# Bricktricker/gpu-solve

Measured on AMD Instinct MI355X. Metric: MLUPS (Jacobi smoother) + V-cycle wall-time, 512³ fp64; achieved HBM GB/s %peak, higher is better.
Workload: dtype f64

## Files before the change

gpu-solve_amd/csrc/gs_device.hpp:

```cpp
#pragma once
#include <hip/hip_runtime.h>
#include <math.h>

#include <cmath>
#include <stdint.h>
#include <stdlib.h>

#include <map>
#include <mutex>
#include <utility>

#include "gpusolve_hip.h"

#ifdef GS_EXP_NOEXP
#define exp(x) ((x) * 1.0000001)
#endif
#ifdef GS_EXP_NOBAR
#define GS_LDS_BARRIER() __builtin_amdgcn_s_waitcnt(0xc07f)
#else
#define GS_LDS_BARRIER()                                                                                               \
    do {                                                                                                               \
        __builtin_amdgcn_s_waitcnt(0xc07f);                                                                            \
        __builtin_amdgcn_s_barrier();                                                                                  \
    } while (0)
#endif

namespace {

constexpr int WAVE = 64;

constexpr bool newtonish(int m) { return m == GS_NEWTON || m == GS_NEWTON_B; }
constexpr int base_mode(int m) { return m == GS_NEWTON_G ? GS_NEWTON_B : m; }

template <bool B>
struct BoolC {
    __device__ static constexpr bool get() { return B; }
};
struct RtBool {
    bool b;
    __device__ bool get() const { return b; }
};

struct Coef {
    double s[7];
    double hh;
    double omega[3];
    double gamma;
    double alpha;
    double preFac;
    int fastdiv;
    int unit;
    int swz;
    int zq;
    int bconst;
    int64_t off[7];
#ifdef GS_EXP_EFIELD
    int64_t efoff;
#endif
};

bool canonical_order(const gs_stencil* S)
{
    static const int cx[7] = {0, 1, -1, 0, 0, 0, 0};
    static const int cy[7] = {0, 0, 0, 1, -1, 0, 0};
    static const int cz[7] = {0, 0, 0, 0, 0, 1, -1};
    for (int i = 0; i < 7; i++)
        if (S->ox[i] != cx[i] || S->oy[i] != cy[i] || S->oz[i] != cz[i]) return false;
    return true;
}

bool valid_stencil(const gs_stencil* S)
{
    for (int i = 0; i < 7; i++)
        if (S->ox[i] < -1 || S->ox[i] > 1 || S->oy[i] < -1 || S->oy[i] > 1 || S->oz[i] < -1 || S->oz[i] > 1)
            return false;
    return true;
}

struct Knobs {
    bool unitStencil, tbxPfd2, pairXh, fitRounds, bigChunks, oneRound, rrLds, zeroQ, newtonXh, specCached;
    int xhSwizzle, midZc, rrZc, rrZcBig, oneRoundMid, rbZc;
    int slabZc, pairZc, rrNr, rrNtu, rrReverse, rrNg, rrDma;
    bool pairFx;
    int fmgNt;
    int64_t pairMinBlocks;
    static int num(const char* name, int dflt)
    {
        const char* e = getenv(name);
        return e && *e ? atoi(e) : dflt;
    }
    Knobs()
        : unitStencil(getenv("GS_NO_UNIT_STENCIL") == nullptr), tbxPfd2(num("GS_TBX_PFD", 2) != 1),
          pairXh(num("GS_PAIR_XH", 1) != 0), fitRounds(num("GS_FIT_ROUNDS", 1) != 0),
          bigChunks(num("GS_PAIR_BIG_CHUNKS", 1) != 0), oneRound(num("GS_PAIR_ONE_ROUND", 1) != 0),
          rrLds(getenv("GS_RR_LDS") != nullptr), zeroQ(getenv("GS_NO_ZERO_Q") == nullptr),
          newtonXh(num("GS_NEWTON_XH", 1) != 0), specCached(num("GS_SPEC_CACHED", 0) != 0),
          xhSwizzle(num("GS_XH_SWIZZLE", 1)), midZc(num("GS_MID_ZC", 0)), rrZc(num("GS_RR_ZC", 0)), rrZcBig(num("GS_RR_ZC_BIG", 0)), oneRoundMid(num("GS_PAIR_ONE_ROUND_MID", 0)), rbZc(num("GS_RB_ZC", 0)), slabZc(num("GS_SLAB_ZC", 0)), pairZc(num("GS_PAIR_ZC", 0)),
          rrNr(num("GS_RR_NR", 0)), rrNtu(num("GS_RR_NTU", 2)), rrReverse(num("GS_RR_REVERSE", 1)), rrNg(num("GS_RR_NG", 0)), rrDma(num("GS_RR_DMA", 0)),
          pairFx(num("GS_PAIR_FX", 1) != 0), fmgNt(num("GS_FMG_NT", -1)),
          pairMinBlocks(num("GS_PAIR_MIN_BLOCKS", 128))
    {
    }
};
const Knobs kKnobs;

#ifdef GS_EXP_EFIELD
int64_t gs_exp_efoff = 0;
#endif

Coef make_coef(const gs_stencil* S, const gs_level* L, double omega, double gamma, int bconst = 0)
{
    Coef k;
    for (int i = 0; i < 7; i++) {
        k.s[i] = S->s[i];
        k.off[i] = S->ox[i] + S->oy[i] * L->ldy + S->oz[i] * L->ldz;
    }
    k.hh = L->h * L->h;
    for (int i = 0; i < 3; i++) k.omega[i] = omega;
    k.gamma = gamma;
    k.alpha = k.hh / S->s[0];
    k.preFac = S->s[0] / k.hh;
    k.fastdiv = k.hh >= 0x1p-120 && k.hh <= 1.0;
    k.unit = kKnobs.unitStencil && (S->s[0] >= 1.0 || S->s[0] <= -1.0);
    for (int i = 1; i < 7; i++) k.unit = k.unit && S->s[i] == -1.0;
    k.swz = kKnobs.xhSwizzle;
    k.zq = kKnobs.zeroQ && std::isnormal(k.hh) && k.hh > 0.0;
    for (int i = 0; i < 7; i++) k.zq = k.zq && std::isfinite(S->s[i]);
    k.bconst = bconst;
#ifdef GS_EXP_EFIELD
    k.efoff = gs_exp_efoff;
#endif
    return k;
}

Coef make_coef_w(const gs_stencil* S, const gs_level* L, const double* omegas, int n, double gamma, int bconst = 0)
{
    Coef k = make_coef(S, L, omegas[0], gamma, bconst);
    for (int i = 1; i < 3; i++) k.omega[i] = omegas[i < n ? i : n - 1];
    return k;
}


__device__ __forceinline__ double hh_recip(double hh)
{
    const double y0 = __builtin_amdgcn_rcp(hh);
    const double y1 = __builtin_fma(y0, __builtin_fma(-hh, y0, 1.0), y0);
    return __builtin_fma(y1, __builtin_fma(-hh, y1, 1.0), y1);
}

__device__ __forceinline__ double div_hh(const Coef& k, double s)
{
    const unsigned e = ((unsigned)__double2hiint(s) >> 20) & 0x7ffu;
    if (k.fastdiv && e - 124u < 1500u) {
        const double y = hh_recip(k.hh);
        const double q = s * y;
        const double r = __builtin_fma(-k.hh, q, s);
        return __builtin_fma(r, y, q);
    }
    return s / k.hh;
}

__device__ __forceinline__ bool div_hh_fast_ok(double s)
{
    const unsigned e = ((unsigned)__double2hiint(s) >> 20) & 0x7ffu;
    return e - 124u < 1500u;
}
template <int N>
__device__ __forceinline__ void div_hh_n(const Coef& k, double (&s)[N])
{
    bool ok = k.fastdiv;
#pragma unroll
    for (int i = 0; i < N; i++) ok &= div_hh_fast_ok(s[i]);
    if (ok) {
        const double y = hh_recip(k.hh);
#pragma unroll
        for (int i = 0; i < N; i++) {
            const double q = s[i] * y;
            const double r = __builtin_fma(-k.hh, q, s[i]);
            s[i] = __builtin_fma(r, y, q);
        }
    } else {
#pragma unroll
// ... 166 lines not shown
    return MODE == GS_NEWTON_B ? 1.0 : exp(w);
}

__device__ __forceinline__ double wave_sum(double x)
{
#pragma unroll
    for (int o = WAVE / 2; o > 0; o >>= 1) x += __shfl_down(x, o, WAVE);
    return x;
}

template <int NWAVES>
__device__ __forceinline__ double block_sum(double x, double* lds, int nw = NWAVES)
{
    const int tid = threadIdx.x + threadIdx.y * blockDim.x;
    x = wave_sum(x);
    if ((tid & (WAVE - 1)) == 0) lds[tid / WAVE] = x;
    __syncthreads();
    double t = 0.0;
    if (tid == 0) {
#pragma unroll
        for (int i = 0; i < NWAVES; i++)
            if (i < nw) t += lds[i];
    }
    return t;
}

template <bool DPP>
__device__ __forceinline__ double lane_from_left(double src, double edge)
{
    if (DPP) {
        const long long s = __double_as_longlong(src), e = __double_as_longlong(edge);
        const int lo = __builtin_amdgcn_update_dpp((int)e, (int)s, 0x138, 0xf, 0xf, false);
        const int hi = __builtin_amdgcn_update_dpp((int)(e >> 32), (int)(s >> 32), 0x138, 0xf, 0xf, false);
        return __longlong_as_double(((long long)hi << 32) | (unsigned)lo);
    } else {
        const double t = __shfl_up(src, 1, WAVE);
        return (threadIdx.x & (WAVE - 1)) == 0 ? edge : t;
    }
}

template <bool DPP>
__device__ __forceinline__ double lane_from_right(double src, double edge)
{
    if (DPP) {
        const long long s = __double_as_longlong(src), e = __double_as_longlong(edge);
        const int lo = __builtin_amdgcn_update_dpp((int)e, (int)s, 0x130, 0xf, 0xf, false);
        const int hi = __builtin_amdgcn_update_dpp((int)(e >> 32), (int)(s >> 32), 0x130, 0xf, 0xf, false);
        return __longlong_as_double(((long long)hi << 32) | (unsigned)lo);
    } else {
        const double t = __shfl_down(src, 1, WAVE);
        return (threadIdx.x & (WAVE - 1)) == WAVE - 1 ? edge : t;
    }
}

__device__ __forceinline__ double uniform_d(double x)
{
    const long long b = __double_as_longlong(x);
    const int lo = __builtin_amdgcn_readfirstlane((int)b), hi = __builtin_amdgcn_readfirstlane((int)(b >> 32));
    return __longlong_as_double(((long long)(unsigned)hi << 32) | (unsigned)lo);
}

__device__ __forceinline__ double2 ld2(const double* __restrict__ p) { return *reinterpret_cast<const double2*>(p); }

typedef double dv2 __attribute__((ext_vector_type(2)));
template <bool NT>
__device__ __forceinline__ double2 ld2s(const double* __restrict__ p)
{
    if (NT) {
        const dv2 t = __builtin_nontemporal_load(reinterpret_cast<const dv2*>(p));
        return make_double2(t.x, t.y);
    }
    return ld2(p);
}
template <bool NT>
__device__ __forceinline__ void st2s(double* __restrict__ p, double a, double b)
{
    if (NT) {
        const dv2 t = {a, b};
        __builtin_nontemporal_store(t, reinterpret_cast<dv2*>(p));
    } else {
        *reinterpret_cast<double2*>(p) = make_double2(a, b);
    }
}

template <bool ZV, bool NT = false>
__device__ __forceinline__ double2 ldv2(const double* __restrict__ p)
{
    if (ZV) return make_double2(0.0, 0.0);
    return ld2s<NT>(p);
}
template <bool ZV>
__device__ __forceinline__ double ldv1(const double* __restrict__ p)
{
    return ZV ? 0.0 : *p;
}

__device__ __forceinline__ int64_t xcd_tile(int64_t b, int64_t nb)
{
    const int64_t q = nb / 8, r = nb % 8, x = b % 8, k = b / 8;
    return (x < r ? x * (q + 1) : r * (q + 1) + (x - r) * q) + k;
}

template <int MODE, int KIND, bool ADD, int RY, int W, bool DPP, bool NT = false, bool XCD = false, bool NTV = false,
          bool ZV = false, bool UN = false>
__global__ __launch_bounds__(WAVE* W) void k_rb(Coef k, const double* __restrict__ v, const double* __restrict__ f,
                                                 const double* __restrict__ w, double* __restrict__ out,
                                                 double* __restrict__ partials, int nx, int ny, int nz, int64_t ldy,
                                                 int64_t ldz, int ZC)
{
    __shared__ double red[W];
    const int lane = threadIdx.x;
    const int wv = __builtin_amdgcn_readfirstlane(threadIdx.y);
    int bx = blockIdx.x, by = blockIdx.y, bz = blockIdx.z;
    int64_t tile = blockIdx.x + gridDim.x * ((int64_t)blockIdx.y + gridDim.y * (int64_t)blockIdx.z);
    if (XCD) {
        const int nbx = (nx + 2 * WAVE - 1) / (2 * WAVE), nby = (ny + RY * W - 1) / (RY * W);
        tile = xcd_tile(blockIdx.x, gridDim.x);
        bx = (int)(tile % nbx);
        by = (int)((tile / nbx) % nby);
        bz = (int)(tile / ((int64_t)nbx * nby));
    }
    const int x0 = 1 + bx * (2 * WAVE);
    const int x = x0 + 2 * lane;
    const int xl = min(x, nx + 1);
    const int y0 = 1 + (by * W + wv) * RY;
    const int zb = 1 + bz * ZC;
    const int ze = min(zb + ZC - 1, nz);
    const int xle = x0 - 1;
    const int xre = min(x0 + 2 * WAVE, nx + 1);
    const bool okx0 = x <= nx, okx1 = x + 1 <= nx;
    const double* fin = (KIND == 2) ? out : f;

    int64_t roff[RY + 2];
#pragma unroll
    for (int r = 0; r < RY + 2; r++) roff[r] = (int64_t)min(y0 - 1 + r, ny + 1) * ldy;

    double2 P[RY], C[RY], NL[2][RY], FL[2][RY], WL[2][RY], HL[2][2];
    double EL[2][RY], ER[2][RY];
    double sumsq = 0.0;
    auto load_slot = [&](const int s, const int64_t z1, const int64_t z2) {
#pragma unroll
        for (int r = 0; r < RY; r++) {
            NL[s][r] = ldv2<ZV, NTV>(v + xl + roff[r + 1] + z2);
            if (KIND != 2 || ADD) FL[s][r] = ld2s<NT>(fin + xl + roff[r + 1] + z1);
            if (newtonish(MODE)) WL[s][r] = ld2(w + xl + roff[r + 1] + z1);
            EL[s][r] = ldv1<ZV>(v + xle + roff[r + 1] + z1);
            ER[s][r] = ldv1<ZV>(v + xre + roff[r + 1] + z1);
        }
        HL[s][0] = ldv2<ZV>(v + xl + roff[0] + z1);
        HL[s][1] = ldv2<ZV>(v + xl + roff[RY + 1] + z1);
    };
    if (zb <= ze) {
        const int64_t zo = (int64_t)zb * ldz;
#pragma unroll
        for (int r = 0; r < RY; r++) {
            P[r] = ldv2<ZV>(v + xl + roff[r + 1] + zo - ldz);
            C[r] = ldv2<ZV>(v + xl + roff[r + 1] + zo);
        }
        load_slot(1, zo, zo + ldz);
    }
    for (int z0 = zb; z0 <= ze; z0 += 2) {
#pragma unroll
        for (int ph = 0; ph < 2; ph++) {
            const int z = z0 + ph;
            const bool real = z <= ze;
            const int cs = ph ^ 1;
// ... 2180 lines not shown
                        }
                    }
                }
            };
            if constexpr (!SPEC) {
                sweeps(RtBool{mir});
            } else {
                if (mir) sweeps(BoolC<true>{});
                else sweeps(BoolC<false>{});
            }
#pragma unroll
            for (int j = 1; j <= RY; j++) {
                V1p[j - 1] = V1c[j];
                if (!RECOMP) Fprev[j - 1] = FL[cs][j];
                if constexpr (RECOMP) {
                    wprev_l[j - 1][wx + WX * wy][lane] = WL[cs][j];
                    fprev_l[j - 1][wx + WX * wy][lane] = FL[cs][j];
                } else if (newtonish(MODE)) {
                    Aprev[j - 1] = Acur[j - 1];
                    Eprev[j - 1] = Ecur[j - 1];
                }
            }
#pragma unroll
            for (int j = 0; j < NV; j++) {
                V1c[j] = V1n[j];
                Vp[j] = Vc[j];
                Vc[j] = VL[cs][j];
            }
            if constexpr (XH) {
                EP = EC;
                if constexpr (EPK) {
                    if (edg) EC = efld(cs, 0);
                } else {
                    EC = EA[cs];
                }
                ES1c = ES1n;
            }
            if (PRO && ph == 1) {
                if constexpr (WLDS) {
                    wsl ^= 1;
                } else {
#pragma unroll
                    for (int r = 0; r < NCR; r++) W0[r] = W1[r];
                    if constexpr (HALF) {
#pragma unroll
                        for (int r = 0; r < NCR; r++) H0[r] = H1[r];
                    }
                }
                xpass(1);
            }
        }
    }
    if (partials) {
        sumsq = wave_sum(sumsq);
        const int wid = wx + WX * wy;
        if (lane == 0) red[wid] = sumsq;
        __syncthreads();
        if (tid == 0) {
            double t = 0.0;
            for (int i = 0; i < 2 * WX; i++) t += red[i];
            partials[tile] = t;
        }
    }
    if constexpr (TS) {
        if (tid == 0) {
            double* t = const_cast<double*>(es) + 4 * tile;
            t[0] = (double)tstart;
            t[1] = (double)wall_clock64();
            t[2] = (double)(blockIdx.x + (int64_t)gridDim.x * blockIdx.y);
            t[3] = (double)(unsigned)__builtin_amdgcn_s_getreg((31 << 11) | 4);
        }
    }
}

constexpr int TBY_RY = 2, TBY_RY_NEWTON = 2, TBY_WX = 4, TB_RY_B = 2, TB_WX_B = 8;
constexpr int tby_pfd(int mode) { return mode == GS_LINEAR ? 2 : 1; }
bool tbx_pfd2() { return kKnobs.tbxPfd2; }

#ifdef GS_EXP_T3_CHAIN
#define GS_T3_ZP(n, c) c
#else
#define GS_T3_ZP(n, c) n
#endif
template <bool UN, bool FX, bool DB>
__global__ __launch_bounds__(WAVE* TBY_WX * 2) void k_tb3y(Coef k, const double* __restrict__ v,
                                                           const double* __restrict__ f, double* __restrict__ out,
                                                           int nx, int ny, int nz, int64_t ldy, int64_t ldz, int ZC)
{
    constexpr int MODE = GS_LINEAR, RY = TBY_RY, WXMAX = TBY_WX;
    static_assert(RY == 2, "k_tb3y: two rows per y-wave (the boundary tests below name the rows)");
    constexpr int N0 = RY + 2;
    constexpr int N1 = RY + 1;
    constexpr int NE = N0 + N1 + RY;
    constexpr int B1 = DB ? 2 : 1, B2 = DB ? N1 : 1, B3 = 1;
    __shared__ double edge[2][2][WXMAX + 2][2][NE];
    __shared__ double2 yrow[2][2][WXMAX][3][WAVE];
    __shared__ double2 f1_l[2][N1][2 * WXMAX][WAVE];
    __shared__ double2 f2_l[RY][2 * WXMAX][WAVE];
    __shared__ double2 s1p_l[N1][2 * WXMAX][WAVE];
    __shared__ double2 s2p_l[RY][2 * WXMAX][WAVE];
    const int lane = threadIdx.x;
    const int wy = __builtin_amdgcn_readfirstlane(threadIdx.z);
    const int WX = blockDim.y;
    const int wx = __builtin_amdgcn_readfirstlane(threadIdx.y);
    const int wid = wx + WXMAX * wy;
    const int tid = threadIdx.x + WAVE * (threadIdx.y + WX * threadIdx.z);
    for (int i = tid; i < 2 * 2 * (WXMAX + 2) * 2 * NE; i += WAVE * WX * 2) (&edge[0][0][0][0][0])[i] = 0.0;
    __syncthreads();
    const int64_t tile = xcd_tile(blockIdx.x + (int64_t)gridDim.x * blockIdx.y, (int64_t)gridDim.x * gridDim.y);
    const int x = 1 + wx * (2 * WAVE) + 2 * lane;
    const int xl = min(x, nx + 1);
    const bool bx0 = !FX && x > nx, bx1 = !FX && x + 1 > nx;
    const bool okx0 = FX || x <= nx, okx1 = FX || x + 1 <= nx;
    const int y0 = 1 + (int)(tile % gridDim.x) * (2 * RY);
    const int zb = 1 + (int)(tile / gridDim.x) * ZC;
    const int ze = min(zb + ZC - 1, nz);
    const bool mir = wy != 0;
    auto yof = [&](int j) { return mir ? y0 + 2 * RY - j : y0 - 1 + j; };

    int64_t roff[RY + 3];
    bool rowc[RY + 3];
#pragma unroll
    for (int j = -2; j <= RY; j++) {
        const int y = yof(j);
        roff[j + 2] = (int64_t)min(max(y, 0), ny + 1) * ldy;
        rowc[j + 2] = y >= 1 && y <= ny;
    }
    const bool in1 = rowc[1] && rowc[2] && rowc[3] && rowc[4];
    const bool in2 = rowc[2] && rowc[3] && rowc[4];
    auto planeok = [&](int z) { return z >= 1 && z <= nz; };
    auto cz = [&](int z) { return min(max(z, 0), nz + 1); };
    auto at = [&](const double* base, int j, int z) { return base + xl + roff[j + 2] + (int64_t)z * ldz; };

    double2 Vp[N0], Vc[N0], VL[2][N0], FL[2][N0], HL[2];
    double2 S1a[N0], S1c[N0], S2c[N1];
#pragma unroll
    for (int i = 0; i < N0; i++) S1a[i] = S1c[i] = make_double2(0.0, 0.0);
#pragma unroll
    for (int i = 0; i < N1; i++) {
        S2c[i] = make_double2(0.0, 0.0);
        f1_l[0][i][wid][lane] = f1_l[1][i][wid][lane] = make_double2(0.0, 0.0);
        s1p_l[i][wid][lane] = make_double2(0.0, 0.0);
    }
#pragma unroll
    for (int i = 0; i < RY; i++) {
        f2_l[i][wid][lane] = make_double2(0.0, 0.0);
        s2p_l[i][wid][lane] = make_double2(0.0, 0.0);
    }
    auto load_slot = [&](const int s, const int z, const int zv) {
        HL[s] = ld2(at(v, -2, z));
#pragma unroll
        for (int i = 0; i < N0; i++) VL[s][i] = ld2(at(v, i - 1, zv));
#pragma unroll
        for (int i = 0; i < N0; i++) FL[s][i] = ld2(at(f, i - 1, z));
    };
#pragma unroll
    for (int i = 0; i < N0; i++) {
        Vp[i] = ld2(at(v, i - 1, cz(zb - 3)));
        Vc[i] = ld2(at(v, i - 1, cz(zb - 2)));
    }
    load_slot(1, cz(zb - 2), cz(zb - 1));
    for (int z0 = zb - 3; z0 <= ze + 2; z0 += 2) {
#pragma unroll
        for (int ph = 0; ph < 2; ph++) {
            const int z = z0 + ph;
            const int cs = ph ^ 1;
            load_slot(ph, cz(z + 2), cz(z + 3));
            if (lane == 0) {
#pragma unroll
                for (int i = 0; i < N0; i++) edge[ph][wy][wx + 1][0][i] = Vc[i].x;
#pragma unroll
                for (int i = 0; i < N1; i++) edge[ph][wy][wx + 1][0][N0 + i] = S1c[i + 1].x;
#pragma unroll
                for (int i = 0; i < RY; i++) edge[ph][wy][wx + 1][0][N0 + N1 + i] = S2c[i + 1].x;
            }
            if (lane == WAVE - 1) {
#pragma unroll
                for (int i = 0; i < N0; i++) edge[ph][wy][wx + 1][1][i] = Vc[i].y;
#pragma unroll
                for (int i = 0; i < N1; i++) edge[ph][wy][wx + 1][1][N0 + i] = S1c[i + 1].y;
#pragma unroll
                for (int i = 0; i < RY; i++) edge[ph][wy][wx + 1][1][N0 + N1 + i] = S2c[i + 1].y;
            }
            yrow[ph][wy][wx][0][lane] = Vc[N0 - 1];
            yrow[ph][wy][wx][1][lane] = S1c[N0 - 1];
            yrow[ph][wy][wx][2][lane] = S2c[N1 - 1];
            GS_LDS_BARRIER();
            const double* const CL = edge[ph][wy][wx][1];
            const double* const CR = edge[ph][wy][wx + 2][0];
            const double2 vY = yrow[ph][wy ^ 1][wx][0][lane];
            const double2 s1Y = yrow[ph][wy ^ 1][wx][1][lane];
            const double2 s2Y = yrow[ph][wy ^ 1][wx][2][lane];

            auto row_sums = [&](auto mirc, const double2 c, const double2 lm, const double2 lp, const double2 zm,
                                const double2 zp, const double el, const double er, double& q0, double& q1) {
                constexpr bool M = decltype(mirc)::get();
                const double2 ym = M ? lp : lm, yp = M ? lm : lp;
                const double xm0 = lane_from_left<true>(c.y, el);
                const double xp1 = lane_from_right<true>(c.x, er);
                if constexpr (UN) {
                    q0 = stencil_sum<true>(k, c.x, c.y, xm0, yp.x, ym.x, zp.x, zm.x);
                    q1 = stencil_sum<true>(k, c.y, xp1, c.x, yp.y, ym.y, zp.y, zm.y);
                } else {
                    q0 = stencil_sum_in_order(k, c.x, c.y, xm0, yp.x, ym.x, zp.x, zm.x);
                    q1 = stencil_sum_in_order(k, c.y, xp1, c.x, yp.y, ym.y, zp.y, zm.y);
                }
            };
            auto row_finish = [&](const double om, const double2 c, const double q0, const double q1, const double2 fv) {
                const double a0 = op_finish<MODE>(k, q0, c.x, 0.0);
                const double a1 = op_finish<MODE>(k, q1, c.y, 0.0);
                return make_double2(jacobi_update<MODE>(k, c.x, fv.x - a0, 0.0, om),
                                    jacobi_update<MODE>(k, c.y, fv.y - a1, 0.0, om));
            };
            auto kept = [&](const bool keep, const double2 c, const double2 n) {
                return make_double2((keep || bx0) ? c.x : n.x, (keep || bx1) ? c.y : n.y);
            };
            double2 S1n[N0], S2n[N1], F1[N1];
            const bool pz0 = planeok(z + 1), pz1 = planeok(z - 1);
            static_assert(N0 % B1 == 0 && N1 % B2 == 0 && RY % B3 == 0, "whole division batches");
            auto sweep1 = [&](auto mirc) {
#pragma unroll
                for (int b = 0; b < N0; b += B1) {
                    double q[2 * B1];
#pragma unroll
                    for (int i = b; i < b + B1; i++)
#ifdef GS_EXP_T3_FLIGHT
                        row_sums(mirc, Vc[i], i == 0 ? Vc[1] : Vc[i - 1], i == N0 - 1 ? vY : Vc[i + 1], Vp[i], Vp[i],
                                 CL[i], CR[i], q[2 * (i - b)], q[2 * (i - b) + 1]);
#else
                        row_sums(mirc, Vc[i], i == 0 ? HL[cs] : Vc[i - 1], i == N0 - 1 ? vY : Vc[i + 1], Vp[i], VL[cs][i],
                                 CL[i], CR[i], q[2 * (i - b)], q[2 * (i - b) + 1]);
#endif
                    div_hh_mm(k, q);
#pragma unroll
                    for (int i = b; i < b + B1; i++)
#ifdef GS_EXP_T3_FLIGHT
                        S1n[i] = row_finish(k.omega[0], Vc[i], q[2 * (i - b)], q[2 * (i - b) + 1], Vp[i]);
#else
                        S1n[i] = row_finish(k.omega[0], Vc[i], q[2 * (i - b)], q[2 * (i - b) + 1], FL[cs][i]);
#endif
                }
                if (!FX || !pz0 || !in1) {
#pragma unroll
                    for (int i = 0; i < N0; i++) S1n[i] = kept(!pz0 || !rowc[i + 1], Vc[i], S1n[i]);
                }
            };
            auto sweep2 = [&](auto mirc) {
#pragma unroll
                for (int b = 0; b < N1; b += B2) {
                    double q[2 * B2];
#pragma unroll
                    for (int i = b; i < b + B2; i++) {
                        F1[i] = f1_l[ph][i][wid][lane];
                        row_sums(mirc, S1c[i + 1], S1c[i], i == N1 - 1 ? s1Y : S1c[i + 2], s1p_l[i][wid][lane],
                                 GS_T3_ZP(S1a[i + 1], S1c[i + 1]),
                                 CL[N0 + i], CR[N0 + i], q[2 * (i - b)], q[2 * (i - b) + 1]);
                    }
                    div_hh_mm(k, q);
#pragma unroll
                    for (int i = b; i < b + B2; i++)
                        S2n[i] = row_finish(k.omega[1], S1c[i + 1], q[2 * (i - b)], q[2 * (i - b) + 1], F1[i]);
                }
                if (!FX || !pz1 || !in2) {
#pragma unroll
                    for (int i = 0; i < N1; i++) S2n[i] = kept(!pz1 || !rowc[i + 2], S1c[i + 1], S2n[i]);
                }
            };
            auto sweep3 = [&](auto mirc) {
                if (z - 2 >= zb && z - 2 <= ze) {
                    const int64_t zo = (int64_t)(z - 2) * ldz;
#pragma unroll
                    for (int b = 1; b <= RY; b += B3) {
                        double q[2 * B3];
                        double2 fv[B3];
#pragma unroll
                        for (int j = b; j < b + B3; j++) {
                            fv[j - b] = f2_l[j - 1][wid][lane];
                            row_sums(mirc, S2c[j], S2c[j - 1], j == RY ? s2Y : S2c[j + 1], s2p_l[j - 1][wid][lane],
                                     GS_T3_ZP(S2n[j], S2c[j]), CL[N0 + N1 + j - 1], CR[N0 + N1 + j - 1], q[2 * (j - b)],
                                     q[2 * (j - b) + 1]);
                        }
                        div_hh_mm(k, q);
#pragma unroll
                        for (int j = b; j < b + B3; j++) {
                            const double2 o = row_finish(k.omega[2], S2c[j], q[2 * (j - b)], q[2 * (j - b) + 1], fv[j - b]);
                            if (yof(j) <= ny) {
                                double* qo = out + x + roff[j + 2] + zo;
                                if (okx1) st2s<true>(qo, o.x, o.y);
                                else if (okx0) *qo = o.x;
                            }
                        }
                    }
                }
            };
            if (mir) sweep2(BoolC<true>{}), sweep3(BoolC<true>{});
            else sweep2(BoolC<false>{}), sweep3(BoolC<false>{});
#pragma unroll
            for (int j = 1; j <= RY; j++) {
                s2p_l[j - 1][wid][lane] = S2c[j];
                f2_l[j - 1][wid][lane] = F1[j];
            }
#pragma unroll
            for (int i = 0; i < N1; i++) {
                S2c[i] = S2n[i];
                s1p_l[i][wid][lane] = S1c[i + 1];
            }
#pragma unroll
            for (int i = 0; i < N0; i++) S1c[i] = S1a[i];
            if (mir) sweep1(BoolC<true>{});
            else sweep1(BoolC<false>{});
#pragma unroll
            for (int i = 0; i < N1; i++) f1_l[ph][i][wid][lane] = FL[cs][i + 1];
#pragma unroll
            for (int i = 0; i < N0; i++) {
                S1a[i] = S1n[i];
                Vp[i] = Vc[i];
                Vc[i] = VL[cs][i];
            }
        }
    }
}

bool xh_enabled() { return kKnobs.pairXh; }

int64_t resident_blocks(const void* fn, int threads)
{
    static std::mutex m;
    static std::map<std::pair<const void*, int>, int64_t> cache;
    std::lock_guard<std::mutex> lk(m);
    const auto key = std::make_pair(fn, threads);
    auto it = cache.find(key);
    if (it != cache.end()) return it->second;
    int per = 0, dev = 0, cus = 0;
    if (hipOccupancyMaxActiveBlocksPerMultiprocessor(&per, fn, threads, 0) != hipSuccess || per < 1) per = 1;
    if (hipGetDevice(&dev) != hipSuccess ||
        hipDeviceGetAttribute(&cus, hipDeviceAttributeMultiprocessorCount, dev) != hipSuccess || cus < 1)
        cus = 256;
    (void)hipGetLastError();
    return cache[key] = (int64_t)per * cus;
}

int fit_chunk(int64_t tiles, int64_t planes, int64_t cap, int lo, int hi, bool even, double halo)
{
    if (!kKnobs.fitRounds || tiles < 1 || planes < 1 || cap < 1) return 0;
    double best = -1.0;
    int bc = 0;
    for (int c = lo; c <= hi; c++) {
        if (even && (c & 1)) continue;
        const int64_t blocks = tiles * ((planes + c - 1) / c);
        if (blocks < cap && bc != 0) continue;
        const int64_t rounds = (blocks + cap - 1) / cap;
        const double score = (double)blocks / (double)(rounds * cap) * c / (c + halo);
        if (score > best) {
            best = score;
            bc = c;
        }
    }
    return bc;
}

template <class K>
void refit_chunks(K* fn, int threads, int64_t planes, int lo, int hi, bool even, double halo, int* zc, dim3* g)
{
    const int c = fit_chunk(g->x, planes, resident_blocks((const void*)fn, threads), lo, hi, even, halo);
    if (c > 0) {
        *zc = c;
        g->y = (unsigned)((planes + c - 1) / c);
    }
}

int64_t device_cus()
{
    static std::mutex m;
    static std::map<int, int64_t> cache;
    int dev = 0;
    if (hipGetDevice(&dev) != hipSuccess) dev = 0;
    std::lock_guard<std::mutex> lk(m);
    auto it = cache.find(dev);
    if (it != cache.end()) return it->second;
    int cus = 0;
    if (hipDeviceGetAttribute(&cus, hipDeviceAttributeMultiprocessorCount, dev) != hipSuccess || cus < 1) cus = 256;
    (void)hipGetLastError();
    return cache[dev] = cus;
}

int slab_zc() { return kKnobs.slabZc; }

int whole_zc() { return kKnobs.pairZc; }
// ... 135 lines not shown
```

gpu-solve_amd/csrc/gs_kernels.hip:

```cpp
#include "gs_device.hpp"

extern "C" {

int gs_field_layout(int64_t nx, int64_t ny, int64_t nz, int64_t* ldy, int64_t* ldz, int64_t* alloc_elems,
                    int64_t* origin_offset)
{
    if (nx < 0 || ny < 0 || nz < 0 || !ldy || !ldz || !alloc_elems || !origin_offset) return GS_EINVAL;
    const int64_t py = ((nx + 2 + 15) / 16) * 16;
    *ldy = py;
    *ldz = py * (ny + 2);
    *origin_offset = 15 + *ldz;
    *alloc_elems = *ldz * (nz + 4) + 32;
    return 0;
}

int gs_rhs_init(const gs_level* L, double* f, int mode, double h0, double gamma, hipStream_t st)
{
    if (bad_level(L) || !f) return GS_EINVAL;
    const dim3 g((unsigned)((L->nx + 2 + 63) / 64), (unsigned)((L->ny + 2 + 3) / 4), (unsigned)(L->nz + 2)), b(64, 4);
    hipLaunchKernelGGL(k_rhs, g, b, 0, st, f, mode, h0, gamma, (int)L->nx, (int)L->ny, (int)L->nz, L->z0, L->ldy,
                       L->ldz);
    return launch_status();
}

// ... 108 lines not shown
        ((xh && tbx_pfd2() && nx % (2 * WAVE * TBY_WX) == 0) || (y2 && nx % (2 * WAVE) == 0))) {
        if (xh)
            hipLaunchKernelGGL((k_tb2y<GS_LINEAR, TBY_RY, TBY_WX, true, false, false, true, 0, 2, true, true, false, 0, true>),
                               g, b, 0, st, k, v_in, f, w, v_out, partials, nx, ny, nz, L->ldy, L->ldz, zc, zlo ? 1 : 0,
                               zhi ? 1 : 0, nullptr, nullptr, 0, 0, 0, 0, 0, nullptr);
        else if (cached)
            hipLaunchKernelGGL((k_tb2y<GS_LINEAR, TBY_RY, TBY_WX, false, false, false, true, 0, 2, false, true, false, 0, true>),
                               g, b, 0, st, k, v_in, f, w, v_out, partials, nx, ny, nz, L->ldy, L->ldz, zc, zlo ? 1 : 0,
                               zhi ? 1 : 0, nullptr, nullptr, 0, 0, 0, 0, 0, nullptr);
        else
            hipLaunchKernelGGL((k_tb2y<GS_LINEAR, TBY_RY, TBY_WX, true, false, false, true, 0, 2, false, true, false, 0, true>),
                               g, b, 0, st, k, v_in, f, w, v_out, partials, nx, ny, nz, L->ldy, L->ldz, zc, zlo ? 1 : 0,
                               zhi ? 1 : 0, nullptr, nullptr, 0, 0, 0, 0, 0, nullptr);
    } else if (mode == GS_NEWTON_B && !zv && y2 && !cached && k.unit && kKnobs.pairFx && nx % (2 * WAVE) == 0) {
        hipLaunchKernelGGL((k_tb2y<GS_NEWTON_B, TBY_RY_NEWTON, TBY_WX, true, false, false, true, 0, 1, false, true, false, 0, true>),
                           g, b, 0, st, k, v_in, f, w, v_out, partials, nx, ny, nz, L->ldy, L->ldz, zc, zlo ? 1 : 0,
                           zhi ? 1 : 0, nullptr, nullptr, 0, 0, 0, 0, 0, nullptr);
    } else if (xh) {
        if (mode == GS_LINEAR) {
            if (zv) GS_TBX(GS_LINEAR, true, 1);
            else if (tbx_pfd2()) GS_TBX(GS_LINEAR, false, 2);
            else GS_TBX(GS_LINEAR, false, 1);
        } else if (mode == GS_NONLINEAR) GS_TBX(GS_NONLINEAR, false, 1);
        else if (mode == GS_NEWTON_B && zv) GS_TBX(GS_NEWTON_B, true, 1);
        else if (mode == GS_NEWTON_B) GS_TBX(GS_NEWTON_B, false, 1);
        else if (zv) GS_TBX(GS_NEWTON, true, 1);
        else GS_TBX(GS_NEWTON, false, 1);
    } else if (y2) {
        if (mode == GS_LINEAR) {
            if (zv) GS_TBY(GS_LINEAR, true);
            else GS_TBY(GS_LINEAR, false);
        } else if (mode == GS_NONLINEAR) GS_TBY(GS_NONLINEAR, false);
        else if (mode == GS_NEWTON_B && zv) GS_TBY(GS_NEWTON_B, true);
        else if (mode == GS_NEWTON_B) GS_TBY(GS_NEWTON_B, false);
        else if (zv) GS_TBY(GS_NEWTON, true);
        else GS_TBY(GS_NEWTON, false);
    } else {
        if (mode == GS_LINEAR) {
            if (zv) GS_TB(GS_LINEAR, true);
            else GS_TB(GS_LINEAR, false);
        } else if (mode == GS_NONLINEAR) GS_TB(GS_NONLINEAR, false);
        else if (mode == GS_NEWTON_B && zv) GS_TB(GS_NEWTON_B, true);
        else if (mode == GS_NEWTON_B) GS_TB(GS_NEWTON_B, false);
        else if (zv) GS_TB(GS_NEWTON, true);
        else GS_TB(GS_NEWTON, false);
    }
#undef GS_TBX
#undef GS_TBX1
#undef GS_TBY
#undef GS_TBY1
#undef GS_TBY2
#undef GS_TB
    return launch_status();
}

int gs_jacobi_sweep3_supported(const gs_stencil* S, const gs_level* L)
{
    int zc;
    dim3 g, b;
    bool y2 = false, xh = false;
    if (!S || bad_level(L) || !valid_stencil(S) || L->z0 != 0) return 0;
    const int q = tb2_plan(S, L, &zc, &g, &b, &y2, GS_LINEAR, &xh);
    return y2 ? q : 0;
}

int gs_jacobi_sweep3(const gs_stencil* S, const gs_level* L, double omega, double gamma, const double* v_in,
                     double* v_out, const double* f, hipStream_t st)
{
    const double omegas[3] = {omega, omega, omega};
    return gs_jacobi_sweep3_w(S, L, omegas, gamma, v_in, v_out, f, st);
}

int gs_jacobi_sweep3_w(const gs_stencil* S, const gs_level* L, const double* omegas, double gamma, const double* v_in,
                       double* v_out, const double* f, hipStream_t st)
{
    int zc;
    dim3 g, b;
    bool y2 = false, xh = false;
    if (!S || !omegas || bad_level(L) || !valid_stencil(S) || L->z0 != 0 || !v_in || !v_out || !f || v_in == v_out ||
        !tb2_plan(S, L, &zc, &g, &b, &y2, GS_LINEAR, &xh) || !y2)
        return GS_EINVAL;
    const Coef k = make_coef_w(S, L, omegas, 3, gamma);
    const int nx = (int)L->nx, ny = (int)L->ny, nz = (int)L->nz;
#define GS_TB3(U, X) hipLaunchKernelGGL((k_tb3y<U, X, U>), g, b, 0, st, k, v_in, f, v_out, nx, ny, nz, L->ldy, L->ldz, zc)
    if (k.unit && kKnobs.pairFx && nx % (2 * WAVE) == 0) GS_TB3(true, true);
    else if (k.unit) GS_TB3(true, false);
    else GS_TB3(false, false);
#undef GS_TB3
    return launch_status();
}

int gs_jacobi_sweep2_prolong_supported(const gs_stencil* S, const gs_level* L, int mode)
{
    int zc;
    dim3 g, b;
    bool y2 = false, xh = false;
    mode = base_mode(mode);
    return !bad_level(L) && valid_stencil(S) && (mode == GS_LINEAR || newtonish(mode)) && L->z0 % 2 == 0 &&
           tb2_plan(S, L, &zc, &g, &b, &y2, mode, &xh, true) && (y2 || xh);
}

int64_t gs_jacobi_sweep2_prolong_ws_elems(const gs_stencil* S, const gs_level* L, int mode)
{
    int zc;
    dim3 g, b;
    bool y2 = false, xh = false;
    mode = base_mode(mode);
    if (!gs_jacobi_sweep2_prolong_supported(S, L, mode) || !tb2_plan(S, L, &zc, &g, &b, &y2, mode, &xh, true) || !xh)
        return 0;
    const int64_t bw = 2 * WAVE * TBY_WX, nb = (L->nx + bw - 1) / bw - 1;
    return nb * (L->nz + 4) * 4 * (L->ny + 2);
}

int gs_jacobi_sweep2_prolong(const gs_stencil* S, const gs_level* L, int mode, double omega, double gamma,
                             const double* v_in, const double* coarse_v, const double* coarse_sub, const gs_level* cl,
                             double* v_out, const double* f, const double* w, int zlo, int zhi, hipStream_t st)
{
    return gs_jacobi_sweep2_prolong_ws(S, L, mode, omega, gamma, v_in, coarse_v, coarse_sub, cl, v_out, f, w, zlo, zhi,
                                       nullptr, 0, st);
}

int gs_jacobi_sweep2_prolong_w(const gs_stencil* S, const gs_level* L, int mode, const double* omegas, double gamma,
                               const double* v_in, const double* coarse_v, const double* coarse_sub,
                               const gs_level* cl, double* v_out, const double* f, const double* w, int zlo, int zhi,
                               hipStream_t st)
{
    return gs_jacobi_sweep2_prolong_ws_w(S, L, mode, omegas, gamma, v_in, coarse_v, coarse_sub, cl, v_out, f, w, zlo,
                                         zhi, nullptr, 0, st);
}

int gs_jacobi_sweep2_prolong_ws(const gs_stencil* S, const gs_level* L, int mode, double omega, double gamma,
                                const double* v_in, const double* coarse_v, const double* coarse_sub,
                                const gs_level* cl, double* v_out, const double* f, const double* w, int zlo, int zhi,
                                double* ws, int64_t ws_elems, hipStream_t st)
{
    const double omegas[2] = {omega, omega};
    return gs_jacobi_sweep2_prolong_ws_w(S, L, mode, omegas, gamma, v_in, coarse_v, coarse_sub, cl, v_out, f, w, zlo,
                                         zhi, ws, ws_elems, st);
}

int gs_jacobi_sweep2_prolong_ws_w(const gs_stencil* S, const gs_level* L, int mode, const double* omegas, double gamma,
                                  const double* v_in, const double* coarse_v, const double* coarse_sub,
                                  const gs_level* cl, double* v_out, const double* f, const double* w, int zlo, int zhi,
                                  double* ws, int64_t ws_elems, hipStream_t st)
{
    int zc;
    dim3 g, b;
    bool y2 = false, xh = false;
    const int bconst = mode == GS_NEWTON_G;
    mode = base_mode(mode);
    const int64_t czoff = cl ? L->z0 / 2 - cl->z0 : 0;
    if (!omegas || !gs_jacobi_sweep2_prolong_supported(S, L, mode) || bad_level(cl) || czoff < 0 || !v_in ||
        !coarse_v || !v_out || !f || v_in == v_out || (mode == GS_NONLINEAR) != (coarse_sub != nullptr) || (newtonish(mode) && !w) ||
        (L->nx + 1) / 2 > cl->nx + 1 || (L->ny + 1) / 2 > cl->ny + 1 || (L->nz + 1) / 2 + czoff > cl->nz + 1 ||
        !tb2_plan(S, L, &zc, &g, &b, &y2, mode, &xh, true))
        return GS_EINVAL;
    const int64_t need = gs_jacobi_sweep2_prolong_ws_elems(S, L, mode);
    if (need > 0 && (!ws || ws_elems < need)) return GS_EINVAL;
    coarse_v += czoff * cl->ldz;
    if (coarse_sub) coarse_sub += czoff * cl->ldz;
    const Coef k = make_coef_w(S, L, omegas, 2, gamma, bconst);
    if (xh && need > 0) {
        const int bw = 2 * WAVE * TBY_WX, nb = (int)((L->nx + bw - 1) / bw - 1);
        hipLaunchKernelGGL(k_pro_strip<false>, dim3((unsigned)((L->ny + 2 + 63) / 64), (unsigned)(L->nz + 4), (unsigned)nb),
                           dim3(256), 0, st, v_in, coarse_v, nullptr, ws, (int)L->nx, (int)L->ny, (int)L->nz, L->ldy,
                           L->ldz, cl->ldy, cl->ldz, bw, zlo ? 1 : 0, zhi ? 1 : 0);
    }
#define GS_TBPF(M, P, U, X, WM, FXV) hipLaunchKernelGGL((k_tb2y<M, newtonish(M) ? TBY_RY_NEWTON : TBY_RY, WM, true, false, false, true, P, 1, X, U, false, 0, FXV>), g, b, 0, st, k, v_in, f, w, v_out, nullptr, (int)L->nx, (int)L->ny, (int)L->nz, L->ldy, L->ldz, zc, zlo ? 1 : 0, zhi ? 1 : 0, coarse_v, coarse_sub, (int)cl->nx, (int)cl->ny, (int)(cl->nz - czoff), cl->ldy, cl->ldz, ws)
    const bool fx = k.unit && kKnobs.pairFx && b.y == TBY_WX && (xh ? L->nx % (2 * WAVE * TBY_WX) == 0 : L->nx % (2 * WAVE) == 0);
#define GS_TBP1(M, P, U, X, WM) do { \
// ... 463 lines not shown
    hipLaunchKernelGGL(k_axpy, dim3((unsigned)blocks), dim3(256), 0, st, y, x, a, n);
    return launch_status();
}

int gs_coarse_cycle_max_levels(void) { return CC_MAXLEV; }

int gs_max_weights(void) { return GS_MAX_WEIGHTS; }

}

static int coarse_cycle(const gs_stencil* S, const gs_coarse_level* lv, int n, int mode, double omega,
                        const double* omegas, double gamma, int pre, int post, hipStream_t st)
{
    mode = base_mode(mode);
    if (!S || !valid_stencil(S) || !lv || n < 1 || n > CC_MAXLEV || mode < GS_LINEAR || mode > GS_NEWTON_B ||
        pre < 0 || post < 0)
        return GS_EINVAL;
    CcPlan P{};
    P.n = n;
    P.pre = pre;
    P.post = post;
    P.weighted = omegas != nullptr;
    for (int i = 0; omegas && i < pre; i++) P.wpre[i] = omegas[i];
    for (int i = 0; omegas && i < post; i++) P.wpost[i] = omegas[pre + i];
    for (int l = 0; l < n; l++) {
        const gs_coarse_level& a = lv[l];
        const gs_level* g = &a.geom;
        if (bad_level(g) || g->z0 != 0 || g->nx < 1 || g->ny < 1 || g->nz < 1 ||
            g->nx * g->ny * g->nz > (int64_t)INT32_MAX || !a.v || !a.v_alt || a.v == a.v_alt || !a.f ||
            (l + 1 < n && !a.r) || (newtonish(mode) && !a.newton_v) ||
            (mode == GS_NONLINEAR && ((l > 0 && !a.rest_v) || a.v_zero)))
            return GS_EINVAL;
        if (l > 0) {
            const gs_level* fg = &lv[l - 1].geom;
            if (g->nx != fg->nx / 2 || g->ny != fg->ny / 2 || g->nz != fg->nz / 2) return GS_EINVAL;
        }
        CcLevel& L = P.L[l];
        L.v = a.v;
        L.va = a.v_alt;
        L.f = a.f;
        L.r = a.r;
        L.rv = a.rest_v;
        L.w = a.newton_v;
        L.ldy = g->ldy;
        L.ldz = g->ldz;
        L.nx = (int)g->nx;
        L.ny = (int)g->ny;
        L.nz = (int)g->nz;
        L.vz = a.v_zero != 0;
        L.k = make_coef(S, g, omega, gamma);
    }
    if (mode == GS_LINEAR) hipLaunchKernelGGL(k_coarse_cycle<GS_LINEAR>, dim3(1), dim3(CC_T), 0, st, P);
    else if (mode == GS_NONLINEAR) hipLaunchKernelGGL(k_coarse_cycle<GS_NONLINEAR>, dim3(1), dim3(CC_T), 0, st, P);
    else if (mode == GS_NEWTON_B) hipLaunchKernelGGL(k_coarse_cycle<GS_NEWTON_B>, dim3(1), dim3(CC_T), 0, st, P);
    else hipLaunchKernelGGL(k_coarse_cycle<GS_NEWTON>, dim3(1), dim3(CC_T), 0, st, P);
    return launch_status();
}

extern "C" {

int gs_coarse_cycle(const gs_stencil* S, const gs_coarse_level* lv, int n, int mode, double omega, double gamma,
                    int pre, int post, hipStream_t st)
{
    return coarse_cycle(S, lv, n, mode, omega, nullptr, gamma, pre, post, st);
}

int gs_coarse_cycle_w(const gs_stencil* S, const gs_coarse_level* lv, int n, int mode, const double* omegas,
                      double gamma, int pre, int post, hipStream_t st)
{
    if (!omegas || pre < 0 || post < 0 || pre > GS_MAX_WEIGHTS || post > GS_MAX_WEIGHTS || pre + post < 1)
        return GS_EINVAL;
    return coarse_cycle(S, lv, n, mode, omegas[0], omegas, gamma, pre, post, st);
}

const char* gs_strerror(int code)
{
    if (code == 0) return "success";
    if (code == GS_EINVAL) return "gpusolve: invalid argument";
    return hipGetErrorString((hipError_t)code);
}

const char* gs_build_info(void)
{
    return "gpusolve_hip v16: LINEAR triples k_tb3y(the pair's whole-row tile, three sweeps per pass, sweep 1 one plane "
           "ahead and last in the step, two load slots, "
           "per-lane f / previous-plane rows in LDS, x-edge values read row by row from LDS into the DPP shift), "
           "pairs k_tb2y(4x2 waves, 2 rows/wave, one round of z-chunks on large levels, LINEAR 2-step prefetch; +prolong; "
           "512-point column blocks for longer rows in every mode; from 64^3 levels; zero-iterate chunks fitted to "
           "resident rounds; zero iterates q = +0; whole-wave rows without range selects (FX); LINEAR loads grouped by "
           "field; x-edge values in VGPRs for LINEAR and the NEWTON_B whole-row plain pair), sweeps k_rb(ry2 w4 zc<=32 "
           "dpp nt), fused residual+restriction (2 coarse rows per block from 2^26 points, descending z-chunks, halo rows "
           "loaded first, non-temporal unshared rows), NEWTON update + "
           "compF (+ level-1 restriction, + the next factor B), NEWTON inner solves on B (GS_NEWTON_B: reciprocal "
           "quotient, shared per pair; GS_NEWTON_G: B = gamma unread), unit-neighbour stencil sums, tiled small levels, "
           "one-workgroup coarse cycle; full-multigrid start (GS_FMG=k, gs_grid_fmg): tricubic gs_fmg_prolong "
           "(k_fmg_prolong: z-march, coarse planes staged in LDS, 16-byte fine stores); fp-contract=off";
}

}

#ifdef GS_EXP_EFIELD
extern "C" void gs_exp_set_efoff(int64_t n) { gs_exp_efoff = n; }
#endif
```

Baseline: 518,000.

## Use scalar row bases with 32-bit lane offsets and keep previous-plane rows in registers

```diff
diff --git a/gpu-solve_amd/csrc/gs_device.hpp b/gpu-solve_amd/csrc/gs_device.hpp
--- a/gpu-solve_amd/csrc/gs_device.hpp
+++ b/gpu-solve_amd/csrc/gs_device.hpp
@@ -81,7 +81,7 @@
     bool unitStencil, tbxPfd2, pairXh, fitRounds, bigChunks, oneRound, rrLds, zeroQ, newtonXh, specCached;
     int xhSwizzle, midZc, rrZc, rrZcBig, oneRoundMid, rbZc;
     int slabZc, pairZc, rrNr, rrNtu, rrReverse, rrNg, rrDma;
-    bool pairFx;
+    bool pairFx, t3Saddr;
     int fmgNt;
     int64_t pairMinBlocks;
     static int num(const char* name, int dflt)
@@ -97,7 +97,7 @@
           newtonXh(num("GS_NEWTON_XH", 1) != 0), specCached(num("GS_SPEC_CACHED", 0) != 0),
           xhSwizzle(num("GS_XH_SWIZZLE", 1)), midZc(num("GS_MID_ZC", 0)), rrZc(num("GS_RR_ZC", 0)), rrZcBig(num("GS_RR_ZC_BIG", 0)), oneRoundMid(num("GS_PAIR_ONE_ROUND_MID", 0)), rbZc(num("GS_RB_ZC", 0)), slabZc(num("GS_SLAB_ZC", 0)), pairZc(num("GS_PAIR_ZC", 0)),
           rrNr(num("GS_RR_NR", 0)), rrNtu(num("GS_RR_NTU", 2)), rrReverse(num("GS_RR_REVERSE", 1)), rrNg(num("GS_RR_NG", 0)), rrDma(num("GS_RR_DMA", 0)),
-          pairFx(num("GS_PAIR_FX", 1) != 0), fmgNt(num("GS_FMG_NT", -1)),
+          pairFx(num("GS_PAIR_FX", 1) != 0), t3Saddr(num("GS_T3_SADDR", 1) != 0), fmgNt(num("GS_FMG_NT", -1)),
           pairMinBlocks(num("GS_PAIR_MIN_BLOCKS", 128))
     {
     }
@@ -430,6 +430,32 @@
         *reinterpret_cast<double2*>(p) = make_double2(a, b);
     }
 }
+
+typedef __attribute__((address_space(1))) const dv2 sa_cdv2;
+typedef __attribute__((address_space(1))) dv2 sa_dv2;
+typedef __attribute__((address_space(1))) double sa_d;
+__device__ __forceinline__ uint64_t sa_base(const double* p)
+{
+    uint64_t a = reinterpret_cast<uint64_t>(p);
+    asm("" : "+s"(a));
+    return a;
+}
+__device__ __forceinline__ unsigned sa_lane(unsigned off)
+{
+    asm("" : "+v"(off));
+    return off;
+}
+__device__ __forceinline__ double2 sa_ld2(uint64_t base, unsigned off)
+{
+    const dv2 t = *reinterpret_cast<sa_cdv2*>(base + off);
+    return make_double2(t.x, t.y);
+}
+__device__ __forceinline__ void sa_st2nt(uint64_t base, unsigned off, double a, double b)
+{
+    const dv2 t = {a, b};
+    __builtin_nontemporal_store(t, reinterpret_cast<sa_dv2*>(base + off));
+}
+__device__ __forceinline__ void sa_st1(uint64_t base, unsigned off, double a) { *reinterpret_cast<sa_d*>(base + off) = a; }
 
 template <bool ZV, bool NT = false>
 __device__ __forceinline__ double2 ldv2(const double* __restrict__ p)
@@ -2776,7 +2802,7 @@
 #else
 #define GS_T3_ZP(n, c) n
 #endif
-template <bool UN, bool FX, bool DB>
+template <bool UN, bool FX, bool DB, bool SA>
 __global__ __launch_bounds__(WAVE* TBY_WX * 2) void k_tb3y(Coef k, const double* __restrict__ v,
                                                            const double* __restrict__ f, double* __restrict__ out,
                                                            int nx, int ny, int nz, int64_t ldy, int64_t ldz, int ZC)
@@ -2786,7 +2812,8 @@
     constexpr int N0 = RY + 2;
     constexpr int N1 = RY + 1;
     constexpr int NE = N0 + N1 + RY;
-    constexpr int B1 = DB ? 2 : 1, B2 = DB ? N1 : 1, B3 = 1;
+    constexpr int B1 = DB ? (SA ? N0 : 2) : 1, B2 = DB ? N1 : 1, B3 = 1;
+    constexpr bool RS = SA;
     __shared__ double edge[2][2][WXMAX + 2][2][NE];
     __shared__ double2 yrow[2][2][WXMAX][3][WAVE];
     __shared__ double2 f1_l[2][N1][2 * WXMAX][WAVE];
@@ -2825,33 +2852,44 @@
     auto planeok = [&](int z) { return z >= 1 && z <= nz; };
     auto cz = [&](int z) { return min(max(z, 0), nz + 1); };
     auto at = [&](const double* base, int j, int z) { return base + xl + roff[j + 2] + (int64_t)z * ldz; };
+    unsigned xo = 8u * (unsigned)xl;
+    auto ldrow = [&](const double* base, int j, int z) {
+        if constexpr (SA) return sa_ld2(sa_base(base + roff[j + 2] + (int64_t)z * ldz), xo);
+        else return ld2(at(base, j, z));
+    };
 
     double2 Vp[N0], Vc[N0], VL[2][N0], FL[2][N0], HL[2];
     double2 S1a[N0], S1c[N0], S2c[N1];
+    double2 S1p[N1], S2p[RY], F2[RY];
 #pragma unroll
     for (int i = 0; i < N0; i++) S1a[i] = S1c[i] = make_double2(0.0, 0.0);
 #pragma unroll
     for (int i = 0; i < N1; i++) {
         S2c[i] = make_double2(0.0, 0.0);
         f1_l[0][i][wid][lane] = f1_l[1][i][wid][lane] = make_double2(0.0, 0.0);
-        s1p_l[i][wid][lane] = make_double2(0.0, 0.0);
+        if constexpr (RS) S1p[i] = make_double2(0.0, 0.0);
+        else s1p_l[i][wid][lane] = make_double2(0.0, 0.0);
     }
 #pragma unroll
     for (int i = 0; i < RY; i++) {
-        f2_l[i][wid][lane] = make_double2(0.0, 0.0);
-        s2p_l[i][wid][lane] = make_double2(0.0, 0.0);
+        if constexpr (RS) {
+            S2p[i] = F2[i] = make_double2(0.0, 0.0);
+        } else {
+            f2_l[i][wid][lane] = make_double2(0.0, 0.0);
+            s2p_l[i][wid][lane] = make_double2(0.0, 0.0);
+        }
     }
     auto load_slot = [&](const int s, const int z, const int zv) {
-        HL[s] = ld2(at(v, -2, z));
-#pragma unroll
-        for (int i = 0; i < N0; i++) VL[s][i] = ld2(at(v, i - 1, zv));
-#pragma unroll
-        for (int i = 0; i < N0; i++) FL[s][i] = ld2(at(f, i - 1, z));
+        HL[s] = ldrow(v, -2, z);
+#pragma unroll
+        for (int i = 0; i < N0; i++) VL[s][i] = ldrow(v, i - 1, zv);
+#pragma unroll
+        for (int i = 0; i < N0; i++) FL[s][i] = ldrow(f, i - 1, z);
     };
 #pragma unroll
     for (int i = 0; i < N0; i++) {
-        Vp[i] = ld2(at(v, i - 1, cz(zb - 3)));
-        Vc[i] = ld2(at(v, i - 1, cz(zb - 2)));
+        Vp[i] = ldrow(v, i - 1, cz(zb - 3));
+        Vc[i] = ldrow(v, i - 1, cz(zb - 2));
     }
     load_slot(1, cz(zb - 2), cz(zb - 1));
     for (int z0 = zb - 3; z0 <= ze + 2; z0 += 2) {
@@ -2859,6 +2897,7 @@
         for (int ph = 0; ph < 2; ph++) {
             const int z = z0 + ph;
             const int cs = ph ^ 1;
+            if constexpr (SA) xo = sa_lane(xo);
             load_slot(ph, cz(z + 2), cz(z + 3));
             if (lane == 0) {
 #pragma unroll
@@ -2946,7 +2985,8 @@
 #pragma unroll
                     for (int i = b; i < b + B2; i++) {
                         F1[i] = f1_l[ph][i][wid][lane];
-                        row_sums(mirc, S1c[i + 1], S1c[i], i == N1 - 1 ? s1Y : S1c[i + 2], s1p_l[i][wid][lane],
+                        row_sums(mirc, S1c[i + 1], S1c[i], i == N1 - 1 ? s1Y : S1c[i + 2],
+                                 RS ? S1p[i] : s1p_l[i][wid][lane],
                                  GS_T3_ZP(S1a[i + 1], S1c[i + 1]),
                                  CL[N0 + i], CR[N0 + i], q[2 * (i - b)], q[2 * (i - b) + 1]);
                     }
@@ -2969,8 +3009,9 @@
                         double2 fv[B3];
 #pragma unroll
                         for (int j = b; j < b + B3; j++) {
-                            fv[j - b] = f2_l[j - 1][wid][lane];
-                            row_sums(mirc, S2c[j], S2c[j - 1], j == RY ? s2Y : S2c[j + 1], s2p_l[j - 1][wid][lane],
+                            fv[j - b] = RS ? F2[j - 1] : f2_l[j - 1][wid][lane];
+                            row_sums(mirc, S2c[j], S2c[j - 1], j == RY ? s2Y : S2c[j + 1],
+                                     RS ? S2p[j - 1] : s2p_l[j - 1][wid][lane],
                                      GS_T3_ZP(S2n[j], S2c[j]), CL[N0 + N1 + j - 1], CR[N0 + N1 + j - 1], q[2 * (j - b)],
                                      q[2 * (j - b) + 1]);
                         }
@@ -2979,9 +3020,16 @@
                         for (int j = b; j < b + B3; j++) {
                             const double2 o = row_finish(k.omega[2], S2c[j], q[2 * (j - b)], q[2 * (j - b) + 1], fv[j - b]);
                             if (yof(j) <= ny) {
-                                double* qo = out + x + roff[j + 2] + zo;
-                                if (okx1) st2s<true>(qo, o.x, o.y);
-                                else if (okx0) *qo = o.x;
+                                if constexpr (SA) {
+                                    xo = sa_lane(xo);
+                                    const uint64_t qb = sa_base(out + roff[j + 2] + zo);
+                                    if (okx1) sa_st2nt(qb, xo, o.x, o.y);
+                                    else if (okx0) sa_st1(qb, xo, o.x);
+                                } else {
+                                    double* qo = out + x + roff[j + 2] + zo;
+                                    if (okx1) st2s<true>(qo, o.x, o.y);
+                                    else if (okx0) *qo = o.x;
+                                }
                             }
                         }
                     }
@@ -2991,13 +3039,19 @@
             else sweep2(BoolC<false>{}), sweep3(BoolC<false>{});
 #pragma unroll
             for (int j = 1; j <= RY; j++) {
-                s2p_l[j - 1][wid][lane] = S2c[j];
-                f2_l[j - 1][wid][lane] = F1[j];
+                if constexpr (RS) {
+                    S2p[j - 1] = S2c[j];
+                    F2[j - 1] = F1[j];
+                } else {
+                    s2p_l[j - 1][wid][lane] = S2c[j];
+                    f2_l[j - 1][wid][lane] = F1[j];
+                }
             }
 #pragma unroll
             for (int i = 0; i < N1; i++) {
                 S2c[i] = S2n[i];
-                s1p_l[i][wid][lane] = S1c[i + 1];
+                if constexpr (RS) S1p[i] = S1c[i + 1];
+                else s1p_l[i][wid][lane] = S1c[i + 1];
             }
 #pragma unroll
             for (int i = 0; i < N0; i++) S1c[i] = S1a[i];
diff --git a/gpu-solve_amd/csrc/gs_kernels.hip b/gpu-solve_amd/csrc/gs_kernels.hip
--- a/gpu-solve_amd/csrc/gs_kernels.hip
+++ b/gpu-solve_amd/csrc/gs_kernels.hip
@@ -214,10 +214,17 @@
         return GS_EINVAL;
     const Coef k = make_coef_w(S, L, omegas, 3, gamma);
     const int nx = (int)L->nx, ny = (int)L->ny, nz = (int)L->nz;
-#define GS_TB3(U, X) hipLaunchKernelGGL((k_tb3y<U, X, U>), g, b, 0, st, k, v_in, f, v_out, nx, ny, nz, L->ldy, L->ldz, zc)
-    if (k.unit && kKnobs.pairFx && nx % (2 * WAVE) == 0) GS_TB3(true, true);
-    else if (k.unit) GS_TB3(true, false);
-    else GS_TB3(false, false);
+#define GS_TB3(U, X, A)                                                                                                \
+    hipLaunchKernelGGL((k_tb3y<U, X, U, A>), g, b, 0, st, k, v_in, f, v_out, nx, ny, nz, L->ldy, L->ldz, zc)
+#define GS_TB3A(U, X)                                                                                                  \
+    do {                                                                                                               \
+        if (kKnobs.t3Saddr) GS_TB3(U, X, true);                                                                        \
+        else GS_TB3(U, X, false);                                                                                      \
+    } while (0)
+    if (k.unit && kKnobs.pairFx && nx % (2 * WAVE) == 0) GS_TB3A(true, true);
+    else if (k.unit) GS_TB3A(true, false);
+    else GS_TB3(false, false, false);
+#undef GS_TB3A
 #undef GS_TB3
     return launch_status();
 }
@@ -847,9 +854,10 @@
 
 const char* gs_build_info(void)
 {
-    return "gpusolve_hip v16: LINEAR triples k_tb3y(the pair's whole-row tile, three sweeps per pass, sweep 1 one plane "
-           "ahead and last in the step, two load slots, "
-           "per-lane f / previous-plane rows in LDS, x-edge values read row by row from LDS into the DPP shift), "
+    return "gpusolve_hip v17: LINEAR triples k_tb3y(the pair's whole-row tile, three sweeps per pass, sweep 1 one plane "
+           "ahead and last in the step, two load slots, scalar row bases + 32-bit lane offsets, "
+           "previous-plane rows in registers, per-lane f in LDS, x-edge values read row by row from LDS into the DPP "
+           "shift), "
            "pairs k_tb2y(4x2 waves, 2 rows/wave, one round of z-chunks on large levels, LINEAR 2-step prefetch; +prolong; "
            "512-point column blocks for longer rows in every mode; from 64^3 levels; zero-iterate chunks fitted to "
            "resident rounds; zero iterates q = +0; whole-wave rows without range selects (FX); LINEAR loads grouped by "
```

New measurement: 539,600, median of 6. +4.2%, better.
